# 3DTopia/3DTopia-XL

Hardware: AMD Instinct MI355X
Metric: DiT denoise-steps/sec (N_prim=2048) + samples/sec @25-step DDIM (higher is better)
Workload: dtype f16

## Files before the change

3dtopia-xl_amd/_lib.py:

```python
from __future__ import annotations

import ctypes as C
import os
from typing import Optional

_HERE = os.path.dirname(os.path.abspath(__file__))
LIB_PATH = os.environ.get("PRIMX_LIB") or os.path.join(_HERE, "csrc", "libprimx_hip.so")

F32, F16, BF16 = 0, 1, 2
ACT_NONE, ACT_GELU_TANH, ACT_GELU_ERF = 0, 1, 2
HEADS_ROWS, HEADS_VT, HEADS_KROWS = 0, 1, 2
ABI_VERSION = 35

_p, _i, _l, _f, _d = C.c_void_p, C.c_int, C.c_int64, C.c_float, C.c_double



class DitBlockFold(C.Structure):
    _fields_ = [(n, _p) for n in ("w_q", "b_q", "w_cproj", "b_cproj", "w_qkv", "w_proj", "b_proj", "w_fc1", "w_fc2", "b_fc2",
                                  "Kc", "Vc", "Kb", "Vb", "uv_q", "uv_qkv", "uv_fc1",
                                  "carry_q", "carry_cproj", "carry_fc1", "carry_fc2")] + \
               [(n, _l) for n in ("carry_q_bytes", "carry_cproj_bytes", "carry_fc1_bytes", "carry_fc2_bytes")]


# ... 32 lines not shown
    "primx_linear_gate_residual": [_p, _p, _p, _p, _l, _p, _i, _i, _i, _i, _i, _p, _l, _p],
    "primx_linear_gate_residual_ln": [_p, _p, _p, _p, _l, _p, _i, _i, _i, _i, _p, _p, _l, _p, _f, _p, _l, _i, _p, _l, _p],
    "primx_ln_sync_timeouts": [],
    "primx_linear_f32out": [_p, _p, _p, _p, _i, _i, _i, _i, _i, _p],
    "primx_row_stats": [_p, _i, _i, _f, _p, _p],
    "primx_linear_gate_residual_fold": [_p, _p, _p, _p, _l, _p, _i, _i, _i, _i, _p, _l, _p, _p, _p, _i, _p, _l, _p],
    "primx_linear_heads_fold": [_p, _p, _i, _i, _i, _i, _i, _i, _i, C.POINTER(_i), C.POINTER(_p), _i, _f, _p, _p, _p, _p, _p, _f,
                                _i, _p, _l, _p],
    "primx_linear_heads_fold_pair": [_p, _p, _i, _i, _i, _i, _i, _i, _i, C.POINTER(_i), C.POINTER(_p), _i, _f, _p, _p, _p, _p, _p, _f,
                                     _p, _p, _p, _i, _i, _i, _i, _i, _i, _i, C.POINTER(_i), C.POINTER(_p), _i, _f, _i, _p],
    "primx_linear_f32out_group": [_p, _i, _i, _i, _i, _i, _i, _p],
    "primx_linear_fold": [_p, _p, _p, _i, _i, _i, _i, _p, _p, _p, _p, _p, _f, _i, _p, _l, _p],
    "primx_linear_heads": [_p, _p, _p, _i, _i, _i, _i, _i, _i, _i, C.POINTER(_i), C.POINTER(_p), _i, _i, _i, _f, _i, _p, _l, _p],
    "primx_attention": [_p, _p, _p, _p, _i, _i, _i, _i, _i, _i, _i, _f, _i, _p],
    "primx_attention_bcast": [_p, _p, _p, _p, _i, _i, _i, _i, _i, _i, _i, _f, _p, _p, _i, _i, _i, _p],
    "primx_pack_heads": [_p, _l, _l, _l, _p, _i, _i, _i, _i, _i, _i, _i, _p],
    "primx_cfg_combine": [_p, _p, _i, _l, _f, _p],
    "primx_diffusion_step": [_p, _p, _i, _l, _i, _i, _p, _i, _i, _i, _i, _i, _p, _p, _p, _p],
    "primx_q_sample": [_p, _p, _l, _p, _i, _p, _p],
    "primx_diffusion_reverse_step": [_p, _p, _i, _l, _i, _i, _p, _i, _i, _i, _p, _p, _p],
    "primx_diffusion_step_keep": [_p, _p, _i, _l, _i, _i, _p, _i, _i, _i, _i, _i, _p, _p, _p, _p, _i, _p, _p, _p],
    "primx_groupnorm_silu": [_p, _p, _p, _p, _i, _i, _i, _i, _f, _i, _i, _p],
    "primx_conv3d_k3": [_p, _p, _p, _p, _f, _p, _i, _i, _i, _i, _i, _i, _p],
    "primx_conv3d_s4_pack": [_p, _p, _i, _i, _p],
    "primx_conv3d_s4_packed": [_p, _p, _p, _p, _f, _p, _i, _i, _i, _p],
    "primx_conv3d_s8_pack": [_p, _p, _p, _i, _p],
    "primx_conv3d_s8_fused": [_p, _p, _p, _p, _p, _p, _p, _f, _p, _p, _p, _i, _i, _p],
    "primx_conv3d_s8_packed": [_p, _p, _p, _p, _f, _p, _i, _i, _p],
    "primx_convtranspose_s4_pack": [_p, _p, _i, _p],
    "primx_convtranspose_s4_packed": [_p, _p, _p, _p, _p, _i, _i, _p],
# ... 53 lines not shown
_MESH_ENTRY_POINTS: set = {"primx_mcubes_workspace", "primx_mcubes_count", "primx_mcubes_emit", "primx_noise_filter"}
_TEXBAKE_ENTRY_POINTS: set = {"primx_texbake_labels", "primx_texbake_components_workspace", "primx_texbake_components",
                              "primx_texbake_raster_workspace", "primx_texbake_raster", "primx_texbake_compact",
                              "primx_texbake_fill_workspace", "primx_texbake_fill"}
_MESHCLEAN_ENTRY_POINTS: set = {"primx_meshclean_workspace", "primx_meshclean_merge", "primx_meshclean_faces",
                                "primx_meshclean_components", "primx_meshclean_edges", "primx_meshclean_fans"}
_MESHDECIM_ENTRY_POINTS: set = {"primx_meshdecim_workspace", "primx_meshdecim_edges", "primx_meshdecim_quadrics",
                                "primx_meshdecim_costs", "primx_meshdecim_select", "primx_meshdecim_collapse",
                                "primx_meshdecim_finish", "primx_meshdecim_normals"}
_VAEENC_ENTRY_POINTS: set = {"primx_latent_norm", "primx_enc_conv_in", "primx_conv3d_down_s8c32", "primx_enc_head"}
_EDIT_ENTRY_POINTS: set = {"primx_q_sample", "primx_diffusion_reverse_step", "primx_diffusion_step_keep"}
_FIT_ENTRY_POINTS: set = {"primx_mesh_field_query", "primx_mesh_face_areas", "primx_mesh_surface_points", "primx_fps"}
_REFINE_ENTRY_POINTS: set = {"primx_primsdf_query_backward", "primx_adam_step"}
_RAYMARCH_GRAD_ENTRY_POINTS: set = {"primx_raymarch_backward"}
_MATERIAL_ENTRY_POINTS: set = {"primx_material_sample"}
_AB_ABI_VERSIONS: tuple = (21, 22, 23, 24, 25, 26, 27, 28, 29, 30, 31, 32, 33, 34)
_fold_available: dict = {}
_blocks_call: dict = {}
_kv_ride: dict = {}
_f32out_group: dict = {}
_null_skip: dict = {}

_lib: Optional[C.CDLL] = None


class PrimxError(RuntimeError):
    """A C-ABI entry point returned a non-zero status."""


def load(path: Optional[str] = None) -> C.CDLL:
    global _lib
    if _lib is not None and path is None:
        return _lib
    path = path or LIB_PATH
    if not os.path.exists(path):
        raise RuntimeError(
# ... 33 lines not shown
            continue
        if got < 29 and name in _MESHCLEAN_ENTRY_POINTS:
            continue
        if got < 30 and name in _MESHDECIM_ENTRY_POINTS:
            continue
        if got < 31 and name in _VAEENC_ENTRY_POINTS:
            continue
        if got < 32 and name in _EDIT_ENTRY_POINTS:
            continue
        if got < 33 and name in _FIT_ENTRY_POINTS:
            continue
        if got < 34 and name in _REFINE_ENTRY_POINTS:
            continue
        if got < 35 and name in _RAYMARCH_GRAD_ENTRY_POINTS:
            continue
        if ab and (name in _MATERIAL_ENTRY_POINTS or name == "primx_dit_blocks_fold_features") and not hasattr(lib, name):
            continue
        fn = getattr(lib, name)
        fn.argtypes = argtypes
        fn.restype = _RESTYPES.get(name, C.c_int)
    _fold_available[path] = got >= 23
    _blocks_call[path] = got >= 24
    _kv_ride[path] = got >= 25
    _f32out_group[path] = got >= 26
    _null_skip[path] = got >= 35 and hasattr(lib, "primx_dit_blocks_fold_features") and bool(lib.primx_dit_blocks_fold_features() & 1)
    if path == LIB_PATH:
        _lib = lib
    return lib


def fold_available() -> bool:
    load()
    return _fold_available.get(LIB_PATH, False)


def blocks_call_available() -> bool:
    load()
    return _blocks_call.get(LIB_PATH, False)


def kv_ride_available() -> bool:
    load()
    return _kv_ride.get(LIB_PATH, False)


def f32out_group_available() -> bool:
    load()
    return _f32out_group.get(LIB_PATH, False)


def null_skip_available() -> bool:
    load()
    return _null_skip.get(LIB_PATH, False)


def check(status: int, name: str) -> None:
    if status != 0:
        msg = load().primx_last_error()
        raise PrimxError(f"{name} failed ({status}): {msg.decode() if msg else '?'}")
```

3dtopia-xl_amd/csrc/attention.hip:

```cpp
#include <stdio.h>
#include <stdlib.h>
#include <type_traits>

#include "common.h"

namespace {

constexpr int QPAD = 128;
constexpr int NW = 8;
constexpr int BQ = 32 * NW;
constexpr int BKV = 64;
constexpr int NSTAGE = 3;
constexpr float RESCALE_THR = 8.0f;
constexpr int WAITCNT_LGKM0 = 0xC07F;

template <typename V8>
__device__ __forceinline__ V8 ldg16(const void* ptr) {
    typedef __attribute__((address_space(1))) const V8 GV8;
    return *reinterpret_cast<GV8*>(reinterpret_cast<uintptr_t>(ptr));
}

__device__ unsigned long long g_attn_prof[8];

template <int DT, int KSTEPS, int DTILES, int KMASK, int PROF = 0>
__global__ __launch_bounds__(64 * NW, 1) void attn_kernel(const typename T16<DT>::S* __restrict__ Qp,
                                                          const typename T16<DT>::S* __restrict__ Kp,
                                                          const typename T16<DT>::S* __restrict__ Vt,
                                                          typename T16<DT>::S* __restrict__ out, int H, int nq, int nq_pad,
                                                          int nkv, int nkv_pad, int dh, float c ,
                                                          const typename T16<DT>::S* __restrict__ Kb,
                                                          const typename T16<DT>::S* __restrict__ Vb, int b_from, int nkv_pad_b) {
    using S = typename T16<DT>::S;
    using V8 = typename T16<DT>::V8;
    using V4 = typename T16<DT>::V4;
    typedef __attribute__((address_space(1))) const void GV;
    typedef __attribute__((address_space(3))) void LV;
    constexpr int DP = 16 * KSTEPS;
    constexpr int KROW = DP + 8;
    constexpr int VR = 32 * DTILES;
    constexpr int KT = BKV * KROW;
    constexpr int VT_ = VR * 64;
    constexpr int BUF = KT + VT_;
    constexpr int NK = KT / 512;
    constexpr int NV = DP / 8;
    constexpr int HW = NW / 2;
    constexpr int NSLOT = ((NK > NV ? NK : NV) + HW - 1) / HW;
    static_assert(KT % 512 == 0, "K tile must be whole DMA instructions");
    __shared__ __attribute__((aligned(16))) S smem[NSTAGE * BUF];

    const int tid = threadIdx.x, lane = tid & 63;
    const int wave = __builtin_amdgcn_readfirstlane(tid >> 6);
    const int grp = wave / HW, rw = wave % HW;
    const int l31 = lane & 31, hi = lane >> 5;
    int bh = blockIdx.x, qt = blockIdx.y;
    if ((gridDim.x & 7) == 0) {
        const int id = blockIdx.x + gridDim.x * blockIdx.y, l = id >> 3, j = l / (int)gridDim.y;
        qt = l - j * (int)gridDim.y;
        bh = (id & 7) + 8 * j;
    }
    const int q0 = qt * BQ;
    const bool bcast = (bh / H) >= b_from;
    const int kvp = bcast ? nkv_pad_b : nkv_pad;
    const S* Kbase = bcast ? Kb + (int64_t)(bh % H) * kvp * KROW : Kp + (int64_t)bh * kvp * KROW;
    const S* Vbase = bcast ? Vb + (int64_t)(bh % H) * DP * kvp : Vt + (int64_t)bh * DP * kvp;

    if (VR > DP) {
        for (int i = tid; i < (VR - DP) * 64; i += 64 * NW) {
#pragma unroll
            for (int stg = 0; stg < NSTAGE; ++stg) smem[stg * BUF + KT + DP * 64 + i] = (S)0.f;
        }
    }

    constexpr bool QCOL = !KMASK && (16 * KSTEPS - 3 >= 16 * (KSTEPS - 1) + 8);
    V8 qf[KSTEPS];
    auto load_q = [&]() {
        const S* qrow = Qp + ((int64_t)bh * nq_pad + min(q0 + wave * 32 + l31, nq_pad - 1)) * DP + hi * 8;
#pragma unroll
        for (int s = 0; s < KSTEPS; ++s) qf[s] = ldg16<V8>(qrow + s * 16);
        if (QCOL) {
#pragma unroll
            for (int s = 0; s < KSTEPS; ++s)
#pragma unroll
                for (int e = 0; e < 8; ++e) qf[s][e] = (S)((float)qf[s][e] * c);
        }
    };
    const int dq = dh - 16 * (KSTEPS - 1) - 8 * hi;
    auto set_q_cols = [&](float m) {
        const S mh = (S)(-m);
        const S ml = (S)(-m - (float)mh);
#pragma unroll
        for (int e = 0; e < 8; ++e) {
            if (e == dq) qf[KSTEPS - 1][e] = (S)1.0f;
            if (e == dq + 1) qf[KSTEPS - 1][e] = mh;
            if (e == dq + 2) qf[KSTEPS - 1][e] = ml;
        }
    };

    const int ntiles = (nkv + BKV - 1) / BKV;
    const int n_pc = grp ? NV : NK, per = (n_pc + HW - 1) / HW;
    const int run_first = min(rw * per, n_pc - 1);
    const int run_len = max(min(per, n_pc - rw * per), 1);
    const int64_t piece_stride = grp ? (int64_t)8 * kvp : 512;
    const int tile_stride = grp ? BKV : KT;
    const S* role_base = grp ? Vbase : Kbase;
    const int v_lrow = lane >> 3, v_lc = lane & 7;
    const int lane_off0 = grp ? v_lrow * kvp + ((v_lc ^ ((v_lrow >> 1) & 7)) * 8) : lane * 8;
    const int lane_off1 = grp ? v_lrow * kvp + ((v_lc ^ ((4 + (v_lrow >> 1)) & 7)) * 8) : lane * 8;
    const bool ragged = (nkv & (BKV - 1)) != 0;
    auto tile_at = [&](int tile) {
        const int tl = min(tile, ntiles - 1);
        return bcast ? ((ragged && tl == ntiles - 1) ? 1 : 0) : tl;
    };
    auto issue_run = [&](int tile, int stage) {
        const S* tb = role_base + (int64_t)tile_at(tile) * tile_stride;
#pragma unroll
        for (int i = 0; i < NSLOT; ++i) {
            const int pc = run_first + min(i, run_len - 1);
            const S* src = tb + pc * piece_stride + ((pc & 1) ? lane_off1 : lane_off0);
            __builtin_amdgcn_global_load_lds((GV*)(uintptr_t)src, (LV*)(smem + stage * BUF + (grp * NK + pc) * 512), 16, 0, 0);
        }
    };
    [[maybe_unused]] auto issue_pair = [&](int jp, int stage) { issue_run(jp + 1 - grp, stage); };

    f32x16 o[DTILES];
#pragma unroll
    for (int t = 0; t < DTILES; ++t)
#pragma unroll
        for (int r = 0; r < 16; ++r) o[t][r] = 0.f;
    float m_run = QCOL ? 0.f : -1e30f, l_run = 0.f;
    f32x16 zero16;
#pragma unroll
    for (int r = 0; r < 16; ++r) zero16[r] = 0.f;

    auto read_k = [&](int stage, V8 (&kf)[2][KSTEPS]) {
        const S* kb = smem + stage * BUF + l31 * KROW + hi * 8;
#pragma unroll
        for (int kt = 0; kt < 2; ++kt)
#pragma unroll
            for (int s = 0; s < KSTEPS; ++s) kf[kt][s] = *reinterpret_cast<const V8*>(kb + kt * 32 * KROW + s * 16);
    };
    auto read_v = [&](int stage, int half, V8 (&vf)[DTILES][2]) {
        const S* vb = smem + stage * BUF + KT + l31 * 64;
        const int sw = (l31 >> 1) & 7;
#pragma unroll
        for (int t = 0; t < DTILES; ++t)
#pragma unroll
            for (int k2 = 0; k2 < 2; ++k2)
                vf[t][k2] = *reinterpret_cast<const V8*>(vb + t * 32 * 64 + (((4 * half + 2 * k2 + hi) ^ sw) * 8));
    };
    auto fence_lds = [&]() {
        __builtin_amdgcn_s_waitcnt(WAITCNT_LGKM0);
        __builtin_amdgcn_sched_barrier(0);
    };
    auto qk = [&](const V8 (&kf)[2][KSTEPS], int t, f32x16 (&sc)[2]) {
#pragma unroll
        for (int s = 0; s < KSTEPS; ++s)
#pragma unroll
// ... 44 lines not shown
                        pb[k2][e + u] = (S)pvv;
                    }
                }
            }
    };

#define PRIMX_ATTN_WAITB_N(NF)                                                                                     \
    do {                                                                                                           \
        __builtin_amdgcn_sched_barrier(0);                          \
        __builtin_amdgcn_s_waitcnt(((NF) & 15) | 0x70 | (((NF) >> 4) << 14));            \
        asm volatile("s_barrier" ::: "memory");                                                                    \
        __builtin_amdgcn_sched_barrier(0);                             \
    } while (0)
#define PRIMX_ATTN_WAITB() PRIMX_ATTN_WAITB_N(NFLY)
    constexpr int NFLY = NSLOT * (NSTAGE - 2);
    constexpr int NFLY_L = 0;
    unsigned long long pt = 0, pl = 0, pm = 0, pw = 0, pn = 0, pl_dma = 0, pl_rd = 0;
    auto stamp = [&](unsigned long long& acc) {
        if (PROF) {
            const unsigned long long now = __builtin_readcyclecounter();
            acc += now - pt;
            pt = now;
        }
    };
    [[maybe_unused]] V8 pb0_l[2];
    auto fold_max = [&](f32x16 (&sc)[2], bool first) {
        float mx = fmaxf(sc[0][0], sc[1][0]);
#pragma unroll
        for (int r = 1; r < 16; ++r) mx = fmaxf(fmaxf(mx, sc[0][r]), sc[1][r]);
        {
            const auto sw = __builtin_amdgcn_permlane32_swap(__float_as_uint(mx), __float_as_uint(mx), false, false);
// ... 65 lines not shown
#pragma unroll
                for (int kt = 0; kt < 2; ++kt)
#pragma unroll
                    for (int r = 0; r < 16; ++r)
                        if (kbase + kt * 32 + (r & 3) + 8 * (r >> 2) >= nkv) sn[kt][r] = -1e30f;
            }
        }
        issue_pair(jp, st_refill);
        probs(sc[1], mc, psum, pb1);
        fence_lds();
        pv(vf1, pb1);
        if (KMASK) l_run += psum;
        __builtin_amdgcn_s_setprio(0);
    };

    if (!grp) issue_run(0, NSTAGE - 1);
#pragma unroll
    for (int pr = 0; pr < NSTAGE - 1; ++pr) issue_pair(pr, pr);
    load_q();
    if (QCOL) set_q_cols(0.f);
    f32x16 sA[2], sB[2];
    PRIMX_ATTN_WAITB();
    {
        V8 kf0[2][KSTEPS];
        read_k(NSTAGE - 1, kf0);
        fence_lds();
        asm volatile("s_barrier" ::: "memory");
        qk(kf0, 0, sA);
    }
    if (PROF) pt = __builtin_readcyclecounter();
    int st = 0, st_free = NSTAGE - 1;
    V8 kf[2][KSTEPS], vf0[DTILES][2], vf1[DTILES][2];
    int j = 0;
    for (; j + 1 < ntiles; j += 2) {
        if (grp) { PRIMX_ATTN_WAITB(); stamp(pw); }
        seg_light(st, st_free, j + NSTAGE - 1, sA, kf, vf0, vf1, j == 0);
        stamp(pl);
        PRIMX_ATTN_WAITB_N(NFLY_L);
        stamp(pw);
        seg_matrix(st, j + 1, sA, sB, kf, vf0, vf1, j + NSTAGE - 1, st_free);
        stamp(pm);
        if (!grp) { PRIMX_ATTN_WAITB(); stamp(pw); }
        st_free = st;
        st = (st == NSTAGE - 1) ? 0 : st + 1;
        if (grp) { PRIMX_ATTN_WAITB(); stamp(pw); }
        seg_light(st, st_free, j + NSTAGE, sB, kf, vf0, vf1, false);
        stamp(pl);
        PRIMX_ATTN_WAITB_N(NFLY_L);
        stamp(pw);
        seg_matrix(st, min(j + 2, ntiles - 1), sB, sA, kf, vf0, vf1, j + NSTAGE, st_free);
        stamp(pm);
        if (!grp) { PRIMX_ATTN_WAITB(); stamp(pw); }
        st_free = st;
        st = (st == NSTAGE - 1) ? 0 : st + 1;
        if (PROF) pn += 2;
    }
    if (j < ntiles) {
        if (grp) PRIMX_ATTN_WAITB();
        seg_light(st, st_free, j + NSTAGE - 1, sA, kf, vf0, vf1, j == 0);
        PRIMX_ATTN_WAITB_N(NFLY_L);
        seg_matrix(st, ntiles - 1, sA, sB, kf, vf0, vf1, j + NSTAGE - 1, st_free);
        if (!grp) PRIMX_ATTN_WAITB();
    }
    __builtin_amdgcn_s_waitcnt(0x0070);
#undef PRIMX_ATTN_WAITB
#undef PRIMX_ATTN_WAITB_N
    if (PROF && lane == 0) {
        atomicAdd(&g_attn_prof[0], pl); atomicAdd(&g_attn_prof[1], pm); atomicAdd(&g_attn_prof[2], pw);
        atomicAdd(&g_attn_prof[3], pn); atomicAdd(&g_attn_prof[4], pl_dma); atomicAdd(&g_attn_prof[5], pl_rd);
    }

    float l_tot;
    if (KMASK) {
        l_tot = l_run + __shfl_xor(l_run, 32);
    } else {
        const int rr = dh & 31;
        float lsum = 0.f;
#pragma unroll
        for (int t = 0; t < DTILES; ++t)
#pragma unroll
            for (int r = 0; r < 16; ++r)
                if (t == (dh >> 5) && r == ((rr & 3) + 4 * (rr >> 3))) lsum = o[t][r];
        l_tot = __shfl(lsum, l31 + 32 * ((rr >> 2) & 1));
    }
    const float inv = 1.0f / l_tot;
    const int q = q0 + wave * 32 + l31;
    const int b = bh / H, h = bh - b * H;
    if ((dh & 7) == 0) {
        constexpr int OST = DP + 8;
        static_assert(NW * 32 * OST <= NSTAGE * BUF, "output staging must fit the ring");
        __syncthreads();
        S* ost = smem + wave * (32 * OST);
#pragma unroll
        for (int t = 0; t < DTILES; ++t)
#pragma unroll
            for (int g = 0; g < 4; ++g) {
                const int d = t * 32 + 8 * g + 4 * hi;
                if (d < dh) {
                    V4 v;
#pragma unroll
                    for (int e = 0; e < 4; ++e) v[e] = (S)(o[t][4 * g + e] * inv);
                    *reinterpret_cast<V4*>(ost + l31 * OST + d) = v;
                }
            }
        const int cpr = dh >> 3, npiece = 32 * cpr;
        for (int p = lane; p < npiece; p += 64) {
            const int row = p / cpr, c = p - row * cpr;
            const int qr = q0 + wave * 32 + row;
            if (qr < nq)
                *reinterpret_cast<V8*>(out + ((int64_t)b * nq + qr) * ((int64_t)H * dh) + (int64_t)h * dh + 8 * c) =
                    *reinterpret_cast<const V8*>(ost + row * OST + 8 * c);
        }
        return;
    }
    if (q < nq) {
        S* orow = out + ((int64_t)b * nq + q) * ((int64_t)H * dh) + (int64_t)h * dh;
#pragma unroll
        for (int t = 0; t < DTILES; ++t)
#pragma unroll
            for (int g = 0; g < 4; ++g) {
                const int d = t * 32 + 8 * g + 4 * hi;
                if (d < dh) {
                    V4 v;
// ... 79 lines not shown
            for (int g = 0; g < 4; ++g) {
                V4 w;
#pragma unroll
                for (int e = 0; e < 4; ++e) w[e] = (S)(o[4 * g + e] * inv);
                *reinterpret_cast<V4*>(orow + 8 * g + 4 * hi) = w;
            }
        }
    }
}

static const int g_attn_prof_on = [] {
    const char* e = getenv("PRIMX_ATTN_PROF");
    return e ? atoi(e) : 0;
}();

template <int DT, int KSTEPS, int DTILES, int KMASK>
void launch_attn(const void* Qp, const void* Kp, const void* Vt, void* out, int B, int H, int nq, int nq_pad, int nkv,
                 int nkv_pad, int dh, float c, const void* Kb, const void* Vb, int b_from, int nkv_pad_b, hipStream_t st) {
    using S = typename T16<DT>::S;
    dim3 grid(B * H, (nq_pad + BQ - 1) / BQ);
#define PRIMX_ATTN_LAUNCH(P)                                                                                         \
    hipLaunchKernelGGL((attn_kernel<DT, KSTEPS, DTILES, KMASK, P>), grid, dim3(64 * NW), 0, st, (const S*)Qp,         \
                       (const S*)Kp, (const S*)Vt, (S*)out, H, nq, nq_pad, nkv, nkv_pad, dh, c, (const S*)Kb, (const S*)Vb,  \
                       b_from, nkv_pad_b)
    if constexpr (DT == PRIMX_F16 && KSTEPS == 5) {
        if (g_attn_prof_on) {
            unsigned long long z[8] = {0}, r[8];
            (void)hipMemcpyToSymbol(HIP_SYMBOL(g_attn_prof), z, sizeof(z));
            PRIMX_ATTN_LAUNCH(1);
            (void)hipStreamSynchronize(st);
            (void)hipMemcpyFromSymbol(r, HIP_SYMBOL(g_attn_prof), sizeof(r));
            const double n = r[3] ? (double)r[3] : 1.0;
            fprintf(stderr, "attn segment profile (cycles per step per wave, %llu wave-steps): light %.0f (DMA issue %.0f, LDS read "
                            "issue %.0f, max/rescale %.0f) | matrix %.0f | waits + barriers %.0f | total %.0f\n", r[3],
                    (r[0] + r[4] + r[5]) / n, r[4] / n, r[5] / n, r[0] / n, r[1] / n, r[2] / n, (r[0] + r[1] + r[2] + r[4] + r[5]) / n);
            return;
        }
    }
    PRIMX_ATTN_LAUNCH(0);
#undef PRIMX_ATTN_LAUNCH
}

}

extern "C" int primx_attention(const void* Qp, const void* Kp, const void* Vt, void* out, int B, int H, int nq,
                               int nq_pad, int nkv, int nkv_pad, int dh, float scale, int dtype, void* stream) {
    return primx_attention_bcast(Qp, Kp, Vt, out, B, H, nq, nq_pad, nkv, nkv_pad, dh, scale, nullptr, nullptr, B, 0, dtype, stream);
}

extern "C" int primx_attention_bcast(const void* Qp, const void* Kp, const void* Vt, void* out, int B, int H, int nq, int nq_pad,
                                     int nkv, int nkv_pad, int dh, float scale, const void* Kb, const void* Vb, int b_from,
                                     int nkv_pad_b, int dtype, void* stream) {
    PRIMX_REQUIRE(Qp && out && ((Kp && Vt) || b_from == 0), "primx_attention: null pointer");
    PRIMX_REQUIRE(B > 0 && H > 0 && nq > 0 && nkv > 0, "primx_attention: empty problem");
    PRIMX_REQUIRE(b_from >= 0 && b_from <= B, "primx_attention_bcast: b_from must lie in [0, B] (b_from=%d B=%d)", b_from, B);
    if (b_from < B) {
        const int need = ((nkv % 64) != 0 && nkv > 64) ? 128 : 64;
        PRIMX_REQUIRE(Kb && Vb, "primx_attention_bcast: null broadcast operands");
// ... 6 lines not shown
    if (small64) {
        const float c64 = scale * 1.4426950408889634f;
        PRIMX_DISPATCH_16(dtype, "primx_attention", {
            using S = typename T16<DT>::S;
            hipLaunchKernelGGL((attn64_kernel<DT>), dim3((unsigned)((B * H + 3) / 4)), dim3(256), 0, (hipStream_t)stream, (const S*)Qp,
                               (const S*)Kp, (const S*)Vt, (S*)out, B * H, H, nq, nkv, c64);
        });
        PRIMX_CHECK_LAUNCH("primx_attention");
        return PRIMX_OK;
    }
    PRIMX_REQUIRE(nq_pad >= nq && nq_pad % QPAD == 0, "primx_attention: nq_pad must be a multiple of 128 and >= nq (or 64 for the 64-token, dh = 32 kernel)");
    PRIMX_REQUIRE(b_from == 0 || (nkv_pad >= nkv && nkv_pad % BKV == 0), "primx_attention: nkv_pad must be a multiple of 64 and >= nkv");
    PRIMX_REQUIRE(nq_pad / QPAD <= 65535, "primx_attention: too many query tiles");
    const float c = scale * 1.4426950408889634f;
    hipStream_t st = (hipStream_t)stream;
    PRIMX_DISPATCH_16(dtype, "primx_attention", {
        if (dh == 72) launch_attn<DT, 5, 3, 0>(Qp, Kp, Vt, out, B, H, nq, nq_pad, nkv, nkv_pad, dh, c, Kb, Vb, b_from, nkv_pad_b, st);
        else if (dh == 64) launch_attn<DT, 4, 2, 1>(Qp, Kp, Vt, out, B, H, nq, nq_pad, nkv, nkv_pad, dh, c, Kb, Vb, b_from, nkv_pad_b, st);
        else if (dh == 32) launch_attn<DT, 2, 1, 1>(Qp, Kp, Vt, out, B, H, nq, nq_pad, nkv, nkv_pad, dh, c, Kb, Vb, b_from, nkv_pad_b, st);
        else {
            primx_set_error("primx_attention: unsupported head dim %d (supported: 32, 64, 72)", dh);
            return PRIMX_EINVAL;
        }
    });
    PRIMX_CHECK_LAUNCH("primx_attention");
    return PRIMX_OK;
}
```

3dtopia-xl_amd/ops.py:

```python
from __future__ import annotations

import ctypes as C
import os
from typing import Optional, Sequence, Tuple

import torch

from . import _lib
from ._lib import ACT_GELU_TANH, ACT_NONE, BF16, F16, F32, HEADS_KROWS, HEADS_ROWS, HEADS_VT, check

_DT = {torch.float16: F16, torch.bfloat16: BF16, torch.float32: F32}
BQ, BKV = 128, 64


def dtype_code(dt: torch.dtype) -> int:
    try:
        return _DT[dt]
    except KeyError:
        raise TypeError(f"unsupported dtype {dt}") from None


_launch_dev: Optional[int] = None


# ... 425 lines not shown
                buf[:, :, n:, dh] = KEY_MASK_VALUE
            if DP - dh >= 3:
                buf[:, :, :, dh + 1:dh + 3] = 1.0
    if kind == HEADS_VT and DP > dh:
        k = torch.arange(n, device=device)
        quad = (k >> 2) & 3
        pos = (k & ~15) | ((((quad & 1) << 1) | (quad >> 1)) << 2) | (k & 3)
        buf[:, :, dh].index_fill_(2, pos, 1.0)
    return buf


def bcast_keys(nkv: int) -> int:
    return 64 + (nkv % 64 if nkv > 64 else 0)


def attention(Qp: torch.Tensor, Kp: Optional[torch.Tensor], Vt: Optional[torch.Tensor], nq: int, nkv: int, dh: int, scale: float,
              out: Optional[torch.Tensor] = None, bcast: Optional[Tuple[torch.Tensor, torch.Tensor]] = None) -> torch.Tensor:
    B, H, nq_pad, DP = Qp.shape
    if bcast is not None:
        Kb, Vb = bcast
        b_from = 0 if Kp is None else Kp.shape[0]
        nkv_pad_b = Kb.shape[2]
        if Kb.shape != (1, H, nkv_pad_b, DP + 8) or Vb.shape != (1, H, DP, nkv_pad_b) or not 0 <= b_from < B:
            raise RuntimeError("attention: broadcast operand layout mismatch")
        if Kp is not None and (Vt is None or Vt.shape != (b_from, H, DP, Kp.shape[2]) or Kp.shape[1:] != (H, Kp.shape[2], DP + 8)):
            raise RuntimeError("attention: operand layout mismatch")
        nkv_pad = Kp.shape[2] if Kp is not None else nkv_pad_b
        if out is None:
            out = torch.empty(B, nq, H * dh, dtype=Qp.dtype, device=Qp.device)
        name = f"attn_kernel<{dtype_code(Qp.dtype)}, {padded_head_dim(dh) // 16}, {(dh + 31) // 32}, {int(padded_head_dim(dh) == dh)}, 0>"
        _timed(f"{name} {B * H}x{nq}x{nkv}x{dh}", 4.0 * B * H * nq * nkv * dh, lambda: check(_lib.load().primx_attention_bcast(
            _dev(Qp, "Qp"), _dev(Kp, "Kp", Qp.dtype) if Kp is not None else None, _dev(Vt, "Vt", Qp.dtype) if Kp is not None else None,
            _dev(out, "out", Qp.dtype), B, H, nq, nq_pad, nkv, nkv_pad, dh, scale, _dev(Kb, "Kb", Qp.dtype), _dev(Vb, "Vb", Qp.dtype),
            b_from, nkv_pad_b, dtype_code(Qp.dtype), _stream()), "primx_attention_bcast"))
        return out
    nkv_pad = Kp.shape[2]
    if Vt.shape != (B, H, DP, nkv_pad) or Kp.shape != (B, H, nkv_pad, DP + 8):
        raise RuntimeError("attention: operand layout mismatch")
    if out is None:
        out = torch.empty(B, nq, H * dh, dtype=Qp.dtype, device=Qp.device)
    small = dh == 32 and nq <= 64 and nkv <= 64 and nq_pad == 64 and nkv_pad == 64
    name = f"attn64_kernel<{dtype_code(Qp.dtype)}>" if small else \
        f"attn_kernel<{dtype_code(Qp.dtype)}, {padded_head_dim(dh) // 16}, {(dh + 31) // 32}, {int(padded_head_dim(dh) == dh)}, 0>"
    _timed(f"{name} {B * H}x{nq}x{nkv}x{dh}", 4.0 * B * H * nq * nkv * dh, lambda: check(_lib.load().primx_attention(
        _dev(Qp, "Qp"), _dev(Kp, "Kp", Qp.dtype), _dev(Vt, "Vt", Qp.dtype), _dev(out, "out", Qp.dtype), B, H, nq,
        nq_pad, nkv, nkv_pad, dh, scale, dtype_code(Qp.dtype), _stream()), "primx_attention"))
    return out


def pack_heads(src: torch.Tensor, kind: int, pad_to: int, role: Optional[str] = None) -> torch.Tensor:
    B, M, H, dh = src.shape
    if src.stride(3) != 1 or not src.is_cuda:
        raise RuntimeError("pack_heads: last dim must be contiguous on a HIP device")
    dst = alloc_heads(B, H, M, dh, kind, src.dtype, src.device, pad_to, role)
    m_pad = dst.shape[3] if kind == HEADS_VT else dst.shape[2]
    check(_lib.load().primx_pack_heads(src.data_ptr(), src.stride(0), src.stride(1), src.stride(2), dst.data_ptr(),
                                       kind, B, M, H, dh, m_pad, dtype_code(src.dtype), _stream()), "primx_pack_heads")
    return dst
# ... 399 lines not shown
```

include/primx_hip.h:

```cpp
#ifndef PRIMX_HIP_H
#define PRIMX_HIP_H

#include <stdint.h>

#ifdef __cplusplus
extern "C" {
#endif

#define PRIMX_ABI_VERSION 35

#define PRIMX_F32 0
#define PRIMX_F16 1
#define PRIMX_BF16 2

#define PRIMX_OK 0
#define PRIMX_EINVAL (-1)
#define PRIMX_ELAUNCH (-2)

#define PRIMX_ACT_NONE 0
#define PRIMX_ACT_GELU_TANH 1
#define PRIMX_ACT_GELU_ERF 2

#define PRIMX_HEADS_ROWS 0
#define PRIMX_HEADS_VT 1
// ... 77 lines not shown
int primx_linear_fold(const void* A, const void* W, void* out, int M, int N, int K, int act, const float* part, const float* u,
                      const float* v, const float* center, float* center_out, float eps, int dtype, const void* prefetch,
                      int64_t prefetch_bytes, void* stream);

int primx_linear_heads(const void* A, const void* W, const void* bias, int M, int N, int K, int rows_per_batch,
                       int heads, int dh, int n_seg, const int* kind, void* const* dst, int n_rep,
                       int rep_batches, int n_pad, float scale0, int dtype, const void* prefetch, int64_t prefetch_bytes,
                       void* stream);


int primx_attention(const void* Qp, const void* Kp, const void* Vt, void* out, int B, int H, int nq, int nq_pad,
                    int nkv, int nkv_pad, int dh, float scale, int dtype, void* stream);
int primx_attention_bcast(const void* Qp, const void* Kp, const void* Vt, void* out, int B, int H, int nq, int nq_pad, int nkv,
                          int nkv_pad, int dh, float scale, const void* Kb, const void* Vb, int b_from, int nkv_pad_b, int dtype,
                          void* stream);


typedef struct PrimxDitBlockFold {
    const void *w_q, *b_q, *w_cproj, *b_cproj, *w_qkv, *w_proj, *b_proj, *w_fc1, *w_fc2, *b_fc2;
    const void *Kc, *Vc, *Kb, *Vb;
    const float *uv_q, *uv_qkv, *uv_fc1;
    const void *carry_q, *carry_cproj, *carry_fc1, *carry_fc2;
    int64_t carry_q_bytes, carry_cproj_bytes, carry_fc1_bytes, carry_fc2_bytes;
} PrimxDitBlockFold;

typedef struct PrimxDitForwardFold {
    int dtype, Be, N, D, H, dh, hidden, depth, L, nq_pad, nkv_pad_c, nkv_pad_b, b_from, step, n_steps;
    float ln_eps, scale;
    float* h;
    void *xn, *att, *hid, *Qc, *Qs, *Ks, *Vs;
// ... 205 lines not shown
```

Before: 125.6.

## Split attention KV range across wave groups when grid underfills the device

```diff
diff --git a/3dtopia-xl_amd/_lib.py b/3dtopia-xl_amd/_lib.py
--- a/3dtopia-xl_amd/_lib.py
+++ b/3dtopia-xl_amd/_lib.py
@@ -70,6 +70,8 @@
     "primx_linear_heads": [_p, _p, _p, _i, _i, _i, _i, _i, _i, _i, C.POINTER(_i), C.POINTER(_p), _i, _i, _i, _f, _i, _p, _l, _p],
     "primx_attention": [_p, _p, _p, _p, _i, _i, _i, _i, _i, _i, _i, _f, _i, _p],
     "primx_attention_bcast": [_p, _p, _p, _p, _i, _i, _i, _i, _i, _i, _i, _f, _p, _p, _i, _i, _i, _p],
+    "primx_attention_ksplit_mode": [_i],
+    "primx_attention_ksplit": [_i, _i, _i, _i],
     "primx_pack_heads": [_p, _l, _l, _l, _p, _i, _i, _i, _i, _i, _i, _i, _p],
     "primx_cfg_combine": [_p, _p, _i, _l, _f, _p],
     "primx_diffusion_step": [_p, _p, _i, _l, _i, _i, _p, _i, _i, _i, _i, _i, _p, _p, _p, _p],
@@ -153,12 +155,14 @@
 _REFINE_ENTRY_POINTS: set = {"primx_primsdf_query_backward", "primx_adam_step"}
 _RAYMARCH_GRAD_ENTRY_POINTS: set = {"primx_raymarch_backward"}
 _MATERIAL_ENTRY_POINTS: set = {"primx_material_sample"}
+_ATTN_KSPLIT_ENTRY_POINTS: set = {"primx_attention_ksplit_mode", "primx_attention_ksplit"}
 _AB_ABI_VERSIONS: tuple = (21, 22, 23, 24, 25, 26, 27, 28, 29, 30, 31, 32, 33, 34)
 _fold_available: dict = {}
 _blocks_call: dict = {}
 _kv_ride: dict = {}
 _f32out_group: dict = {}
 _null_skip: dict = {}
+_attn_ksplit: dict = {}
 
 _lib: Optional[C.CDLL] = None
 
@@ -222,7 +226,7 @@
             continue
         if got < 35 and name in _RAYMARCH_GRAD_ENTRY_POINTS:
             continue
-        if ab and (name in _MATERIAL_ENTRY_POINTS or name == "primx_dit_blocks_fold_features") and not hasattr(lib, name):
+        if ab and (name in _MATERIAL_ENTRY_POINTS or name in _ATTN_KSPLIT_ENTRY_POINTS or name == "primx_dit_blocks_fold_features") and not hasattr(lib, name):
             continue
         fn = getattr(lib, name)
         fn.argtypes = argtypes
@@ -232,6 +236,7 @@
     _kv_ride[path] = got >= 25
     _f32out_group[path] = got >= 26
     _null_skip[path] = got >= 35 and hasattr(lib, "primx_dit_blocks_fold_features") and bool(lib.primx_dit_blocks_fold_features() & 1)
+    _attn_ksplit[path] = hasattr(lib, "primx_attention_ksplit")
     if path == LIB_PATH:
         _lib = lib
     return lib
@@ -260,6 +265,11 @@
 def null_skip_available() -> bool:
     load()
     return _null_skip.get(LIB_PATH, False)
+
+
+def attn_ksplit_available() -> bool:
+    load()
+    return _attn_ksplit.get(LIB_PATH, False)
 
 
 def check(status: int, name: str) -> None:
diff --git a/3dtopia-xl_amd/csrc/attention.hip b/3dtopia-xl_amd/csrc/attention.hip
--- a/3dtopia-xl_amd/csrc/attention.hip
+++ b/3dtopia-xl_amd/csrc/attention.hip
@@ -22,7 +22,7 @@
 
 __device__ unsigned long long g_attn_prof[8];
 
-template <int DT, int KSTEPS, int DTILES, int KMASK, int PROF = 0>
+template <int DT, int KSTEPS, int DTILES, int KMASK, int PROF = 0, int KSPLIT = 0>
 __global__ __launch_bounds__(64 * NW, 1) void attn_kernel(const typename T16<DT>::S* __restrict__ Qp,
                                                           const typename T16<DT>::S* __restrict__ Kp,
                                                           const typename T16<DT>::S* __restrict__ Vt,
@@ -44,13 +44,20 @@
     constexpr int NK = KT / 512;
     constexpr int NV = DP / 8;
     constexpr int HW = NW / 2;
-    constexpr int NSLOT = ((NK > NV ? NK : NV) + HW - 1) / HW;
+    constexpr int RWV = KSPLIT ? HW / 2 : HW;
+    constexpr int NSLOT = ((NK > NV ? NK : NV) + RWV - 1) / RWV;
+    constexpr int NRING = KSPLIT ? 2 : 1;
+    constexpr int BQK = KSPLIT ? BQ / 2 : BQ;
     static_assert(KT % 512 == 0, "K tile must be whole DMA instructions");
-    __shared__ __attribute__((aligned(16))) S smem[NSTAGE * BUF];
+    static_assert(NSLOT * (NSTAGE - 2) <= 63, "the DMAs in flight must fit the 6-bit vmcnt field");
+    __shared__ __attribute__((aligned(16))) S smem[NRING * NSTAGE * BUF];
 
     const int tid = threadIdx.x, lane = tid & 63;
     const int wave = __builtin_amdgcn_readfirstlane(tid >> 6);
     const int grp = wave / HW, rw = wave % HW;
+    const int wq = KSPLIT ? rw : wave;
+    const int role = KSPLIT ? rw / RWV : grp, rk = KSPLIT ? rw % RWV : rw;
+    const int ring = KSPLIT ? grp * (NSTAGE * BUF) : 0;
     const int l31 = lane & 31, hi = lane >> 5;
     int bh = blockIdx.x, qt = blockIdx.y;
     if ((gridDim.x & 7) == 0) {
@@ -58,7 +65,7 @@
         qt = l - j * (int)gridDim.y;
         bh = (id & 7) + 8 * j;
     }
-    const int q0 = qt * BQ;
+    const int q0 = qt * BQK;
     const bool bcast = (bh / H) >= b_from;
     const int kvp = bcast ? nkv_pad_b : nkv_pad;
     const S* Kbase = bcast ? Kb + (int64_t)(bh % H) * kvp * KROW : Kp + (int64_t)bh * kvp * KROW;
@@ -67,14 +74,14 @@
     if (VR > DP) {
         for (int i = tid; i < (VR - DP) * 64; i += 64 * NW) {
 #pragma unroll
-            for (int stg = 0; stg < NSTAGE; ++stg) smem[stg * BUF + KT + DP * 64 + i] = (S)0.f;
+            for (int stg = 0; stg < NRING * NSTAGE; ++stg) smem[stg * BUF + KT + DP * 64 + i] = (S)0.f;
         }
     }
 
     constexpr bool QCOL = !KMASK && (16 * KSTEPS - 3 >= 16 * (KSTEPS - 1) + 8);
     V8 qf[KSTEPS];
     auto load_q = [&]() {
-        const S* qrow = Qp + ((int64_t)bh * nq_pad + min(q0 + wave * 32 + l31, nq_pad - 1)) * DP + hi * 8;
+        const S* qrow = Qp + ((int64_t)bh * nq_pad + min(q0 + wq * 32 + l31, nq_pad - 1)) * DP + hi * 8;
 #pragma unroll
         for (int s = 0; s < KSTEPS; ++s) qf[s] = ldg16<V8>(qrow + s * 16);
         if (QCOL) {
@@ -97,15 +104,17 @@
     };
 
     const int ntiles = (nkv + BKV - 1) / BKV;
-    const int n_pc = grp ? NV : NK, per = (n_pc + HW - 1) / HW;
-    const int run_first = min(rw * per, n_pc - 1);
-    const int run_len = max(min(per, n_pc - rw * per), 1);
-    const int64_t piece_stride = grp ? (int64_t)8 * kvp : 512;
-    const int tile_stride = grp ? BKV : KT;
-    const S* role_base = grp ? Vbase : Kbase;
+    const int jbeg = KSPLIT ? (grp ? (ntiles + 1) / 2 : 0) : 0;
+    const int jend = KSPLIT ? (grp ? ntiles : (ntiles + 1) / 2) : ntiles;
+    const int n_pc = role ? NV : NK, per = (n_pc + RWV - 1) / RWV;
+    const int run_first = min(rk * per, n_pc - 1);
+    const int run_len = max(min(per, n_pc - rk * per), 1);
+    const int64_t piece_stride = role ? (int64_t)8 * kvp : 512;
+    const int tile_stride = role ? BKV : KT;
+    const S* role_base = role ? Vbase : Kbase;
     const int v_lrow = lane >> 3, v_lc = lane & 7;
-    const int lane_off0 = grp ? v_lrow * kvp + ((v_lc ^ ((v_lrow >> 1) & 7)) * 8) : lane * 8;
-    const int lane_off1 = grp ? v_lrow * kvp + ((v_lc ^ ((4 + (v_lrow >> 1)) & 7)) * 8) : lane * 8;
+    const int lane_off0 = role ? v_lrow * kvp + ((v_lc ^ ((v_lrow >> 1) & 7)) * 8) : lane * 8;
+    const int lane_off1 = role ? v_lrow * kvp + ((v_lc ^ ((4 + (v_lrow >> 1)) & 7)) * 8) : lane * 8;
     const bool ragged = (nkv & (BKV - 1)) != 0;
     auto tile_at = [&](int tile) {
         const int tl = min(tile, ntiles - 1);
@@ -117,10 +126,10 @@
         for (int i = 0; i < NSLOT; ++i) {
             const int pc = run_first + min(i, run_len - 1);
             const S* src = tb + pc * piece_stride + ((pc & 1) ? lane_off1 : lane_off0);
-            __builtin_amdgcn_global_load_lds((GV*)(uintptr_t)src, (LV*)(smem + stage * BUF + (grp * NK + pc) * 512), 16, 0, 0);
-        }
-    };
-    [[maybe_unused]] auto issue_pair = [&](int jp, int stage) { issue_run(jp + 1 - grp, stage); };
+            __builtin_amdgcn_global_load_lds((GV*)(uintptr_t)src, (LV*)(smem + ring + stage * BUF + (role * NK + pc) * 512), 16, 0, 0);
+        }
+    };
+    [[maybe_unused]] auto issue_pair = [&](int jp, int stage) { issue_run(jp + 1 - role, stage); };
 
     f32x16 o[DTILES];
 #pragma unroll
@@ -133,14 +142,14 @@
     for (int r = 0; r < 16; ++r) zero16[r] = 0.f;
 
     auto read_k = [&](int stage, V8 (&kf)[2][KSTEPS]) {
-        const S* kb = smem + stage * BUF + l31 * KROW + hi * 8;
+        const S* kb = smem + ring + stage * BUF + l31 * KROW + hi * 8;
 #pragma unroll
         for (int kt = 0; kt < 2; ++kt)
 #pragma unroll
             for (int s = 0; s < KSTEPS; ++s) kf[kt][s] = *reinterpret_cast<const V8*>(kb + kt * 32 * KROW + s * 16);
     };
     auto read_v = [&](int stage, int half, V8 (&vf)[DTILES][2]) {
-        const S* vb = smem + stage * BUF + KT + l31 * 64;
+        const S* vb = smem + ring + stage * BUF + KT + l31 * 64;
         const int sw = (l31 >> 1) & 7;
 #pragma unroll
         for (int t = 0; t < DTILES; ++t)
@@ -215,7 +224,7 @@
     } while (0)
 #define PRIMX_ATTN_WAITB() PRIMX_ATTN_WAITB_N(NFLY)
     constexpr int NFLY = NSLOT * (NSTAGE - 2);
-    constexpr int NFLY_L = 0;
+    constexpr int NFLY_L = KSPLIT ? NSLOT : 0;
     unsigned long long pt = 0, pl = 0, pm = 0, pw = 0, pn = 0, pl_dma = 0, pl_rd = 0;
     auto stamp = [&](unsigned long long& acc) {
         if (PROF) {
@@ -311,9 +320,9 @@
         __builtin_amdgcn_s_setprio(0);
     };
 
-    if (!grp) issue_run(0, NSTAGE - 1);
-#pragma unroll
-    for (int pr = 0; pr < NSTAGE - 1; ++pr) issue_pair(pr, pr);
+    if (!role) issue_run(jbeg, NSTAGE - 1);
+#pragma unroll
+    for (int pr = 0; pr < NSTAGE - 1; ++pr) issue_pair(jbeg + pr, pr);
     load_q();
     if (QCOL) set_q_cols(0.f);
     f32x16 sA[2], sB[2];
@@ -323,15 +332,15 @@
         read_k(NSTAGE - 1, kf0);
         fence_lds();
         asm volatile("s_barrier" ::: "memory");
-        qk(kf0, 0, sA);
+        qk(kf0, jbeg, sA);
     }
     if (PROF) pt = __builtin_readcyclecounter();
     int st = 0, st_free = NSTAGE - 1;
     V8 kf[2][KSTEPS], vf0[DTILES][2], vf1[DTILES][2];
-    int j = 0;
-    for (; j + 1 < ntiles; j += 2) {
+    int j = jbeg;
+    for (; j + 1 < jend; j += 2) {
         if (grp) { PRIMX_ATTN_WAITB(); stamp(pw); }
-        seg_light(st, st_free, j + NSTAGE - 1, sA, kf, vf0, vf1, j == 0);
+        seg_light(st, st_free, j + NSTAGE - 1, sA, kf, vf0, vf1, j == jbeg);
         stamp(pl);
         PRIMX_ATTN_WAITB_N(NFLY_L);
         stamp(pw);
@@ -352,12 +361,18 @@
         st = (st == NSTAGE - 1) ? 0 : st + 1;
         if (PROF) pn += 2;
     }
-    if (j < ntiles) {
+    if (j < jend) {
         if (grp) PRIMX_ATTN_WAITB();
-        seg_light(st, st_free, j + NSTAGE - 1, sA, kf, vf0, vf1, j == 0);
+        seg_light(st, st_free, j + NSTAGE - 1, sA, kf, vf0, vf1, j == jbeg);
         PRIMX_ATTN_WAITB_N(NFLY_L);
         seg_matrix(st, ntiles - 1, sA, sB, kf, vf0, vf1, j + NSTAGE - 1, st_free);
         if (!grp) PRIMX_ATTN_WAITB();
+    }
+    if constexpr (KSPLIT) {
+        if (grp && (ntiles & 1)) {
+            asm volatile("s_barrier" ::: "memory");
+            asm volatile("s_barrier" ::: "memory");
+        }
     }
     __builtin_amdgcn_s_waitcnt(0x0070);
 #undef PRIMX_ATTN_WAITB
@@ -367,6 +382,32 @@
         atomicAdd(&g_attn_prof[3], pn); atomicAdd(&g_attn_prof[4], pl_dma); atomicAdd(&g_attn_prof[5], pl_rd);
     }
 
+    if constexpr (KSPLIT) {
+        constexpr int NO = 16 * DTILES;
+        static_assert((NO + 2) * (64 * HW) * 4 <= NSTAGE * BUF * (int)sizeof(S), "the parked partial results must fit ring 0");
+        float* park = reinterpret_cast<float*>(smem) + rw * 64 + lane;
+        __syncthreads();
+        if (grp) {
+#pragma unroll
+            for (int t = 0; t < DTILES; ++t)
+#pragma unroll
+                for (int r = 0; r < 16; ++r) park[(16 * t + r) * (64 * HW)] = o[t][r];
+            park[NO * (64 * HW)] = m_run;
+            if (KMASK) park[(NO + 1) * (64 * HW)] = l_run;
+        }
+        __syncthreads();
+        if (grp) return;
+        const float m1 = park[NO * (64 * HW)];
+        const float m = fmaxf(m_run, m1);
+        const float a0 = __builtin_amdgcn_exp2f(QCOL ? m_run - m : (m_run - m) * c);
+        const float a1 = __builtin_amdgcn_exp2f(QCOL ? m1 - m : (m1 - m) * c);
+#pragma unroll
+        for (int t = 0; t < DTILES; ++t)
+#pragma unroll
+            for (int r = 0; r < 16; ++r) o[t][r] = o[t][r] * a0 + park[(16 * t + r) * (64 * HW)] * a1;
+        if (KMASK) l_run = l_run * a0 + park[(NO + 1) * (64 * HW)] * a1;
+    }
+
     float l_tot;
     if (KMASK) {
         l_tot = l_run + __shfl_xor(l_run, 32);
@@ -381,13 +422,13 @@
         l_tot = __shfl(lsum, l31 + 32 * ((rr >> 2) & 1));
     }
     const float inv = 1.0f / l_tot;
-    const int q = q0 + wave * 32 + l31;
+    const int q = q0 + wq * 32 + l31;
     const int b = bh / H, h = bh - b * H;
     if ((dh & 7) == 0) {
         constexpr int OST = DP + 8;
-        static_assert(NW * 32 * OST <= NSTAGE * BUF, "output staging must fit the ring");
-        __syncthreads();
-        S* ost = smem + wave * (32 * OST);
+        static_assert((KSPLIT ? HW : NW) * 32 * OST <= NSTAGE * BUF, "output staging must fit the ring");
+        if constexpr (!KSPLIT) __syncthreads();
+        S* ost = smem + (KSPLIT ? NSTAGE * BUF : 0) + wq * (32 * OST);
 #pragma unroll
         for (int t = 0; t < DTILES; ++t)
 #pragma unroll
@@ -403,7 +444,7 @@
         const int cpr = dh >> 3, npiece = 32 * cpr;
         for (int p = lane; p < npiece; p += 64) {
             const int row = p / cpr, c = p - row * cpr;
-            const int qr = q0 + wave * 32 + row;
+            const int qr = q0 + wq * 32 + row;
             if (qr < nq)
                 *reinterpret_cast<V8*>(out + ((int64_t)b * nq + qr) * ((int64_t)H * dh) + (int64_t)h * dh + 8 * c) =
                     *reinterpret_cast<const V8*>(ost + row * OST + 8 * c);
@@ -513,34 +554,67 @@
     return e ? atoi(e) : 0;
 }();
 
+static int g_attn_ksplit_mode = [] {
+    const char* e = getenv("PRIMX_ATTN_KSPLIT");
+    return (e && e[0] == '0' && e[1] == 0) ? 0 : -1;
+}();
+
+static int attn_cu_count() {
+    static const int n_cu = [] {
+        int dev = 0, n = 0;
+        (void)hipGetDevice(&dev);
+        if (hipDeviceGetAttribute(&n, hipDeviceAttributeMultiprocessorCount, dev) != hipSuccess || n <= 0) n = 256;
+        return n;
+    }();
+    return n_cu;
+}
+
+static int attn_ksplit(int b_from, int H, int nq_pad, int nkv) {
+    const int ntiles = (nkv + BKV - 1) / BKV;
+    if (g_attn_ksplit_mode == 0 || ntiles < 16) return 0;
+    if (g_attn_ksplit_mode == 1) return 1;
+    return 2LL * b_from * H * ((nq_pad + BQ - 1) / BQ) <= attn_cu_count();
+}
+
 template <int DT, int KSTEPS, int DTILES, int KMASK>
 void launch_attn(const void* Qp, const void* Kp, const void* Vt, void* out, int B, int H, int nq, int nq_pad, int nkv,
-                 int nkv_pad, int dh, float c, const void* Kb, const void* Vb, int b_from, int nkv_pad_b, hipStream_t st) {
+                 int nkv_pad, int dh, float c, const void* Kb, const void* Vb, int b_from, int nkv_pad_b, int ksplit, hipStream_t st) {
     using S = typename T16<DT>::S;
-    dim3 grid(B * H, (nq_pad + BQ - 1) / BQ);
-#define PRIMX_ATTN_LAUNCH(P)                                                                                         \
-    hipLaunchKernelGGL((attn_kernel<DT, KSTEPS, DTILES, KMASK, P>), grid, dim3(64 * NW), 0, st, (const S*)Qp,         \
+    const int bq = ksplit ? BQ / 2 : BQ;
+    dim3 grid(B * H, (nq_pad + bq - 1) / bq);
+#define PRIMX_ATTN_LAUNCH(P, KS)                                                                                     \
+    hipLaunchKernelGGL((attn_kernel<DT, KSTEPS, DTILES, KMASK, P, KS>), grid, dim3(64 * NW), 0, st, (const S*)Qp,     \
                        (const S*)Kp, (const S*)Vt, (S*)out, H, nq, nq_pad, nkv, nkv_pad, dh, c, (const S*)Kb, (const S*)Vb,  \
                        b_from, nkv_pad_b)
     if constexpr (DT == PRIMX_F16 && KSTEPS == 5) {
         if (g_attn_prof_on) {
             unsigned long long z[8] = {0}, r[8];
             (void)hipMemcpyToSymbol(HIP_SYMBOL(g_attn_prof), z, sizeof(z));
-            PRIMX_ATTN_LAUNCH(1);
+            if (ksplit) PRIMX_ATTN_LAUNCH(1, 1);
+            else PRIMX_ATTN_LAUNCH(1, 0);
             (void)hipStreamSynchronize(st);
             (void)hipMemcpyFromSymbol(r, HIP_SYMBOL(g_attn_prof), sizeof(r));
             const double n = r[3] ? (double)r[3] : 1.0;
-            fprintf(stderr, "attn segment profile (cycles per step per wave, %llu wave-steps): light %.0f (DMA issue %.0f, LDS read "
-                            "issue %.0f, max/rescale %.0f) | matrix %.0f | waits + barriers %.0f | total %.0f\n", r[3],
+            fprintf(stderr, "attn segment profile%s (cycles per step per wave, %llu wave-steps): light %.0f (DMA issue %.0f, LDS read "
+                            "issue %.0f, max/rescale %.0f) | matrix %.0f | waits + barriers %.0f | total %.0f\n", ksplit ? " [ksplit]" : "", r[3],
                     (r[0] + r[4] + r[5]) / n, r[4] / n, r[5] / n, r[0] / n, r[1] / n, r[2] / n, (r[0] + r[1] + r[2] + r[4] + r[5]) / n);
             return;
         }
     }
-    PRIMX_ATTN_LAUNCH(0);
+    if (ksplit) PRIMX_ATTN_LAUNCH(0, 1);
+    else PRIMX_ATTN_LAUNCH(0, 0);
 #undef PRIMX_ATTN_LAUNCH
 }
 
 }
+
+extern "C" int primx_attention_ksplit_mode(int mode) {
+    const int was = g_attn_ksplit_mode;
+    g_attn_ksplit_mode = mode < 0 ? -1 : mode > 0 ? 1 : 0;
+    return was;
+}
+
+extern "C" int primx_attention_ksplit(int b_from, int H, int nq_pad, int nkv) { return attn_ksplit(b_from, H, nq_pad, nkv); }
 
 extern "C" int primx_attention(const void* Qp, const void* Kp, const void* Vt, void* out, int B, int H, int nq,
                                int nq_pad, int nkv, int nkv_pad, int dh, float scale, int dtype, void* stream) {
@@ -577,10 +651,11 @@
     PRIMX_REQUIRE(nq_pad / QPAD <= 65535, "primx_attention: too many query tiles");
     const float c = scale * 1.4426950408889634f;
     hipStream_t st = (hipStream_t)stream;
+    const int ks = attn_ksplit(b_from, H, nq_pad, nkv);
     PRIMX_DISPATCH_16(dtype, "primx_attention", {
-        if (dh == 72) launch_attn<DT, 5, 3, 0>(Qp, Kp, Vt, out, B, H, nq, nq_pad, nkv, nkv_pad, dh, c, Kb, Vb, b_from, nkv_pad_b, st);
-        else if (dh == 64) launch_attn<DT, 4, 2, 1>(Qp, Kp, Vt, out, B, H, nq, nq_pad, nkv, nkv_pad, dh, c, Kb, Vb, b_from, nkv_pad_b, st);
-        else if (dh == 32) launch_attn<DT, 2, 1, 1>(Qp, Kp, Vt, out, B, H, nq, nq_pad, nkv, nkv_pad, dh, c, Kb, Vb, b_from, nkv_pad_b, st);
+        if (dh == 72) launch_attn<DT, 5, 3, 0>(Qp, Kp, Vt, out, B, H, nq, nq_pad, nkv, nkv_pad, dh, c, Kb, Vb, b_from, nkv_pad_b, ks, st);
+        else if (dh == 64) launch_attn<DT, 4, 2, 1>(Qp, Kp, Vt, out, B, H, nq, nq_pad, nkv, nkv_pad, dh, c, Kb, Vb, b_from, nkv_pad_b, ks, st);
+        else if (dh == 32) launch_attn<DT, 2, 1, 1>(Qp, Kp, Vt, out, B, H, nq, nq_pad, nkv, nkv_pad, dh, c, Kb, Vb, b_from, nkv_pad_b, ks, st);
         else {
             primx_set_error("primx_attention: unsupported head dim %d (supported: 32, 64, 72)", dh);
             return PRIMX_EINVAL;
diff --git a/3dtopia-xl_amd/ops.py b/3dtopia-xl_amd/ops.py
--- a/3dtopia-xl_amd/ops.py
+++ b/3dtopia-xl_amd/ops.py
@@ -463,6 +463,13 @@
     return 64 + (nkv % 64 if nkv > 64 else 0)
 
 
+def _attn_kernel_name(dtype: torch.dtype, dh: int, b_from: int, H: int, nq_pad: int, nkv: int) -> str:
+    if PROFILE is None:
+        return "attn_kernel"
+    tail = f", {_lib.load().primx_attention_ksplit(b_from, H, nq_pad, nkv)}" if _lib.attn_ksplit_available() else ""
+    return f"attn_kernel<{dtype_code(dtype)}, {padded_head_dim(dh) // 16}, {(dh + 31) // 32}, {int(padded_head_dim(dh) == dh)}, 0{tail}>"
+
+
 def attention(Qp: torch.Tensor, Kp: Optional[torch.Tensor], Vt: Optional[torch.Tensor], nq: int, nkv: int, dh: int, scale: float,
               out: Optional[torch.Tensor] = None, bcast: Optional[Tuple[torch.Tensor, torch.Tensor]] = None) -> torch.Tensor:
     B, H, nq_pad, DP = Qp.shape
@@ -477,7 +484,7 @@
         nkv_pad = Kp.shape[2] if Kp is not None else nkv_pad_b
         if out is None:
             out = torch.empty(B, nq, H * dh, dtype=Qp.dtype, device=Qp.device)
-        name = f"attn_kernel<{dtype_code(Qp.dtype)}, {padded_head_dim(dh) // 16}, {(dh + 31) // 32}, {int(padded_head_dim(dh) == dh)}, 0>"
+        name = _attn_kernel_name(Qp.dtype, dh, b_from, H, nq_pad, nkv)
         _timed(f"{name} {B * H}x{nq}x{nkv}x{dh}", 4.0 * B * H * nq * nkv * dh, lambda: check(_lib.load().primx_attention_bcast(
             _dev(Qp, "Qp"), _dev(Kp, "Kp", Qp.dtype) if Kp is not None else None, _dev(Vt, "Vt", Qp.dtype) if Kp is not None else None,
             _dev(out, "out", Qp.dtype), B, H, nq, nq_pad, nkv, nkv_pad, dh, scale, _dev(Kb, "Kb", Qp.dtype), _dev(Vb, "Vb", Qp.dtype),
@@ -489,8 +496,7 @@
     if out is None:
         out = torch.empty(B, nq, H * dh, dtype=Qp.dtype, device=Qp.device)
     small = dh == 32 and nq <= 64 and nkv <= 64 and nq_pad == 64 and nkv_pad == 64
-    name = f"attn64_kernel<{dtype_code(Qp.dtype)}>" if small else \
-        f"attn_kernel<{dtype_code(Qp.dtype)}, {padded_head_dim(dh) // 16}, {(dh + 31) // 32}, {int(padded_head_dim(dh) == dh)}, 0>"
+    name = f"attn64_kernel<{dtype_code(Qp.dtype)}>" if small else _attn_kernel_name(Qp.dtype, dh, B, H, nq_pad, nkv)
     _timed(f"{name} {B * H}x{nq}x{nkv}x{dh}", 4.0 * B * H * nq * nkv * dh, lambda: check(_lib.load().primx_attention(
         _dev(Qp, "Qp"), _dev(Kp, "Kp", Qp.dtype), _dev(Vt, "Vt", Qp.dtype), _dev(out, "out", Qp.dtype), B, H, nq,
         nq_pad, nkv, nkv_pad, dh, scale, dtype_code(Qp.dtype), _stream()), "primx_attention"))
diff --git a/include/primx_hip.h b/include/primx_hip.h
--- a/include/primx_hip.h
+++ b/include/primx_hip.h
@@ -115,6 +115,8 @@
 int primx_attention_bcast(const void* Qp, const void* Kp, const void* Vt, void* out, int B, int H, int nq, int nq_pad, int nkv,
                           int nkv_pad, int dh, float scale, const void* Kb, const void* Vb, int b_from, int nkv_pad_b, int dtype,
                           void* stream);
+int primx_attention_ksplit_mode(int mode);
+int primx_attention_ksplit(int b_from, int H, int nq_pad, int nkv);
 
 
 typedef struct PrimxDitBlockFold {
```

Result: faster. 127.7 (median of 6 runs) (+1.7%).
